# imaranresearch/LAMMPS-SPHERHARM

Measured on AMD Instinct MI355X. Metric: contact_pairs_per_sec, higher is better.
Workload: dtype f64; 1 GPU; BASELINE configs[1]: 100000 particles/GPU, 1 SH shape(s) L_max=6, dense packed bed (jittered HCP, spacing 1.9 mean radii), n_q=16 (Q=512 nodes/pair), pair_coeff kn=1000 exponent=1.25 (overlap volume + force + torque), inputs resident in HBM; particles_per_gpu=100000, lmax=6, nq=16, rule=sharp, backend=none, half_list_pairs_rank0=579574, contact_pairs_rank0=579574, touching_pairs_rank0=502600, contact_pairs_all_ranks=579574

## Files before the change

### lammps-spherharm_amd/csrc/contact_kernel_azimuth.hpp

```cpp
#pragma once
#include "contact_plan.hpp"
#include "jpoly.hpp"
#include "pair_params.hpp"
#include "pair_rotate.hpp"
#include "ring_tables.hpp"
#include "wave_ops.hpp"

namespace shp {


template <int L, bool NEEDV, int WPP = 1, bool SPEC = false>
__global__ void __launch_bounds__(64 * kMaxWavesPerBlock, SHP_JMIN_WAVES(L, NEEDV, WPP)) pair_contact_azimuth_kernel(const PairParams P)
{
  static_assert(L >= 0, "per-azimuth kernels: compiled orders only");
  constexpr int LJ = L;
  static_assert(!SPEC || (PairSpec<LJ>::nq > 0 && PairSpec<LJ>::wpp == WPP),
                "specialised instances: the orders PairSpec names");
  static_assert(WPP == 1 || WPP == 2, "one or two waves per pair");
  extern __shared__ __attribute__((aligned(16))) unsigned char smem_raw[];
  int lane = threadIdx.x & 63;
  const int wib = __builtin_amdgcn_readfirstlane((int)(threadIdx.x >> 6));
  const int w = P.slot0 + ((WPP == 2) ? (int)blockIdx.x : __builtin_amdgcn_readfirstlane((int)(blockIdx.x * P.waves_per_block)) + wib);
  const int half = (WPP == 2) ? wib : 0;
  const int tid = lane + 64 * half;
  constexpr int NT = 64 * WPP;
  if (w >= P.npairs) return;
  const int LL = L;
  typedef PairSpec<L> Spec;
  const int nq = SPEC ? Spec::nq : P.nq;
  const int P_ring_rows = SPEC ? Spec::rr : P.ring_rows;
  const int P_qcap = SPEC ? Spec::qc : P.qcap;
  constexpr bool CARRY = SHP_CARRY_NODE(L, WPP);
  WaveLdsLayout W = (WPP == 2) ? pair_lds_layout2(LL, P_ring_rows, nq, P_qcap)
                               : wave_lds_layout(LL, P_ring_rows, false, nq, P_qcap);
  if constexpr (WPP == 2) {
    W.qri += half * W.qstride;
    W.qrj += half * W.qstride;
    W.qp += half * W.qstride;
    W.park += half * W.qstride;
  }
  typedef __attribute__((address_space(3))) unsigned char lds_byte_t;
  const unsigned wave_off = (WPP == 2) ? 0u : (unsigned)(wib * P.wave_lds_bytes);
  const unsigned wave_abs = __builtin_amdgcn_readfirstlane((unsigned)(size_t)(lds_byte_t*)smem_raw + wave_off);
#define WAVE_LDS() ((double*)(lds_byte_t*)(size_t)launder_s32(wave_abs))
  double* lw = WAVE_LDS();

  __builtin_amdgcn_s_setprio(3);
  const int* rid = P.rec_i + 4 * (size_t)w;
  constexpr int NSL = ((L + 1) * (L + 1) + NT - 1) / NT;
  double vi[NSL], vj[NSL];
  JPolyPre<LJ> pre;
  const double recv = P.rec[(size_t)kRecStride * w + (lane < kRecUsed ? lane : 0)];
  {
    constexpr int ns = (L + 1) * (L + 1);
#pragma unroll
    for (int t = 0; t < NSL; ++t) {
      const int e = tid + NT * t;
      const int ec = e < ns ? e : 0;
      if constexpr (rot_tiled(L)) {
        const int l = (int)__builtin_amdgcn_sqrtf((float)ec + 0.5f);
        const double* tile = P.rot + (size_t)((2 * w) >> 6) * rot_tile_doubles(L);
        const unsigned at = 64u * (unsigned)(l * l) + (unsigned)((2 * w) & 63) * (unsigned)(2 * l + 1) + (unsigned)(ec - l * l);
        vi[t] = tile[at];
        vj[t] = tile[at + (unsigned)(2 * l + 1)];
      } else {
        const size_t at = (size_t)(2 * w) * rot_row_doubles(L) + ec;
        vi[t] = P.rot[at];
        vj[t] = P.rot[at + rot_row_doubles(L)];
      }
    }
    pre.fetch(P, lane, nq);
  }
  double glt_first = 0.0, glw_first = 0.0;
  glw_first = P.glw[tid < nq ? tid : 0];
  if constexpr (L <= 8 && WPP == 1) {
    const int nr0 = P_ring_rows < nq ? P_ring_rows : nq;
    const int lg0 = ring_poly_map(nr0, L + 1, 64);
    const int kr = lg0 >= 1 ? (lane >> lg0) : lane / (L + 1);
    glt_first = P.glt[kr < nr0 ? kr : nr0 - 1];
  }
  const int status = rid[0];
  if (status == 0) return;
  double s_rho = 0.0, s_rj = 0.0, s_rj2 = 0.0, s_rho2 = 0.0, s_pj = 0.0, s_tol1 = 0.0, s_tol3 = 0.0, s_tiny = 0.0;
  {
    const cdptr rs = launder_uniform(P.rec + (size_t)kRecStride * w);
    s_rho = rs[FR_RHO];
    s_rj = rs[FR_RJ];
    s_rj2 = rs[FR_RJ2];
    s_rho2 = rs[FR_RHO2];
    s_pj = rs[FR_JPJ];
    s_tol1 = rs[FR_JTOL1];
    s_tol3 = rs[FR_JTOL3];
    s_tiny = rs[FR_JTINY];
  }
  const bool centre_in_bj = rid[3] != 0;
  if ((tid >= 12 && tid < 30) || (tid >= 36 && tid < kRecUsed)) lw[frj(tid)] = recv;
  if constexpr (L <= 8 && WPP == 1) lw[W.stash + lane] = glt_first;
#pragma unroll
  for (int t = 0; t < NSL; ++t)
    if (tid + NT * t < (LJ + 1) * (LJ + 1)) {
      lw[W.v0 + tid + NT * t] = vj[t];
      lw[W.v0i + tid + NT * t] = vi[t];
    }
  pair_sync<WPP>();
#if defined(SHP_ABL) && SHP_ABL == 1
  asm volatile("" ::"v"(lw[lane & 31]));
  return;
#endif
  jpoly_build<LJ, WPP>(P, lw, W, lane, nq, pre, glw_first, half);
#if defined(SHP_ABL) && SHP_ABL == 4
  asm volatile("" ::"v"(lw[W.pi + lane]));
  return;
#endif

  const double* fr = WAVE_LDS();

  bool centre_inside = false;
  if (NEEDV && centre_in_bj) {
    const double rho = fr[frj(FR_RHO)];
    const double rj = jpoly_eval<LJ>(fr + W.gh, -1.0, 0.0);
    centre_inside = (rho - rj <= 0.0);
  }

  const int npsi = 2 * nq;
  const unsigned magic = ((1u << 24) + (unsigned)npsi - 1u) / (unsigned)npsi;
  const int per_ring = nq / WPP;
  const unsigned magicr = ((1u << 24) + (unsigned)per_ring - 1u) / (unsigned)per_ring;
  const int nslabs = (nq * per_ring + 63) >> 6;
  const int rowlen = 4 * (LL + 1);

  {
    const int kend0 = (P_ring_rows < nq) ? P_ring_rows : nq;
    cap_frame_rings_poly<LJ, WPP>(P, WAVE_LDS(), W, lane, tid, 0, kend0, fr[frj(FR_HW)], fr[frj(FR_HM)], L <= 8 && WPP == 1);
  }
  bool first_group = true;
  double aV = 0.0, aS0 = 0.0, aS1 = 0.0, aS2 = 0.0, aT0 = 0.0, aT1 = 0.0, aT2 = 0.0;
#if defined(SHP_ABL) && SHP_ABL == 3
  int qhead = 0;
#endif
  int qcount = 0, slab = 0;

  while (slab < nslabs) {
  const int sfirst = slab;
  const int k0 = (int)(((unsigned)(sfirst << 6) * magicr) >> 24);
  const int kend = (k0 + P_ring_rows < nq) ? k0 + P_ring_rows : nq;
  const int slab_end = (kend == nq) ? nslabs : ((kend * per_ring) >> 6);
  if (slab_end <= slab) return;
  __builtin_amdgcn_s_setprio(3);
  {
    double* lr = WAVE_LDS();
    if (!first_group) {
      double* park = lr + W.park + lane;
      park[0] = aT2; park[64] = NEEDV ? aV : aS0;
      if constexpr (WPP == 2) __syncthreads();
      cap_frame_rings_poly<LJ, WPP>(P, lr, W, lane, tid, k0, kend - k0, lr[frj(FR_HW)], lr[frj(FR_HM)], false);
      park = WAVE_LDS() + W.park + lane;
      aT2 = park[0];
      if (NEEDV) aV = park[64]; else aS0 = park[64];
      wave_lds_sync();
    }
    first_group = false;
#if defined(SHP_ABL) && SHP_ABL == 2
    asm volatile("" ::"v"(lr[W.ring + lane]));
    return;
#endif
  }

  auto phase2 = [&](auto dir_c, const int dp, const double dri, const double drj, const unsigned long long mdir)
                    __attribute__((always_inline)) {
    constexpr bool DIR = decltype(dir_c)::value;
    (void)dp; (void)dri; (void)drj; (void)mdir;
    wave_lds_sync();
    fr = WAVE_LDS();
    const int cnt = DIR ? 64 : (qcount < 64 ? qcount : 64);
    const bool active = DIR ? lane_of(mdir) : lane < cnt;
    if constexpr (!DIR) qcount -= cnt;
    const int e = DIR ? 0 : qcount + min(lane, cnt - 1);
#ifdef SHP_STATS
    if (lane == 0) atomicAdd(&P.dbg[4], 1ULL);
    if (active) atomicAdd(&P.dbg[7], 1ULL);
#endif
    int p;
    double ri;
    if constexpr (DIR) {
      p = dp;
      ri = dri;
    } else {
      p = ((const unsigned short*)(fr + W.qp))[e];
      ri = fr[W.qri + e];
    }
    int k = (int)(umul_sel<true>((unsigned)p, magic) >> 24);
    int l = p - mul_sel<true>(k, npsi);
    double omi = active ? fr[frj(FR_WSC)] * fr[W.glw + mul_sel<true>(k, jpoly_row(LJ))] : 0.0;
    double c1 = P.cpsi[l], s1 = P.spsi[l];
    double mu, sig;
    {
      const double* row = fr + W.ring + (k - k0) * rowlen;
      mu = row[1];
      sig = row[3];
    }

    double rin = 0.0;
    if (NEEDV) {
      const double rj0 = DIR ? drj : fr[W.qrj + e];
      double uj0, uj1;
      const int ghrow_ = W.gh + mul_sel<true>(l >= nq ? l - nq : l, jpoly_row(LJ));
      uj0 = mu;
      uj1 = (l >= nq) ? -sig : sig;
      double lo = 0.0, hi = ri, lam, xa = ri, ga, xb = ri, gb;
      {
        double bp, s2i;
        {
          const double rho = s_rho;
          bp = mu * rho;
          const double q0 = fma(ri, uj0, -rho), q1 = ri * uj1;
          s2i = fma(q0, q0, q1 * q1);
        }
        const double rho2l = s_rho2;
        if (!centre_in_bj) lo = bp - sqrt_nr1<true>(fma(bp, bp, -s_pj));
        lam = bp - sqrt_nr1<true>(fma(bp, bp, -(rho2l - rj0 * rj0)));
        if (!(lam > lo && lam < hi)) lam = 0.5 * (lo + hi);
        ga = gb = sqrt_nr1<true>(s2i) - rj0;
      }
      unsigned jrow_addr = wave_abs + 8u * (unsigned)ghrow_;
      unsigned long long mact;
      mact = centre_inside ? 0ULL : (DIR ? mdir : (cnt >= 64 ? ~0ULL : ((1ULL << cnt) - 1ULL)));
      auto iterate = [&](double& xa, double& ga, const double xb, const double gb, const double lam, double& gc,
                         const bool have3) __attribute__((always_inline)) {
#ifdef SHP_STATS
        if (lane == 0) atomicAdd(&P.dbg[5], 1ULL);
        if (lane_of(mact)) atomicAdd(&P.dbg[6], 1ULL);
#endif
        double y0, y1, ss2;
        y0 = fma(lam, uj0, -s_rho);
        y1 = lam * uj1;
        ss2 = fma(y0, y0, y1 * y1);
        const bool z0 = !(ss2 > 0.0);
        const double iv = rsqrt_nr1(ss2);
        double rj;
        jrow_addr = launder_u32(jrow_addr);
        rj = jpoly_eval<LJ>((const double*)(lds_byte_t*)(size_t)jrow_addr, y0 * iv, y1 * iv);
        const double Rjl = s_rj;
        double gl = ss2 * iv - rj;
        if (wave_any(z0)) {
          asm volatile("; rare: a point on x_j");
          gl = z0 ? -Rjl : gl;
        }
        {
          const bool pos = gl >= 0.0;
          lo = pos ? lam : lo;
          hi = pos ? hi : lam;
          const double dbl = gb - gl;
          double ext;
          if (!have3) {
            ext = fma(gl * (lam - xb), rcp_nr1(dbl), lam);
          } else {
            const double dab = ga - gb, dal = ga - gl;
            const double num = fma(xa * gb, gl * dbl, fma(lam * ga, gb * dab, -(xb * ga) * (gl * dal)));
            ext = num * rcp_nr1(dab * dal * dbl);
          }
          const bool inb = ext > lo && ext < hi;
          const bool accept = fabs(gl) <= (have3 ? s_tol3 : s_tol1);
          const bool tiny = hi - lo <= s_tiny;
          double res = ext, nxt = ext;
          unsigned long long mstop = wave_ballot(accept);
          if (mask_any(mact & (wave_ballot(tiny) | ~(wave_ballot(ext > lo) & wave_ballot(ext < hi))))) {
#ifdef SHP_STATS
            if (lane == 0) atomicAdd(&P.dbg[8], 1ULL);
#endif
            double sec = ext, e2 = ext;
            if (have3) {
              const double s2 = fma(gl * (lam - xb), rcp_nr1(dbl), lam);
              const bool fin0 = fabs(ext) <= 1e300;
              sec = (!fin0 || !inb) ? s2 : ext;
              e2 = fin0 ? ext : s2;
            }
            const double mid = 0.5 * (lo + hi);
            double n2 = (e2 > lo && e2 < hi) ? e2 : sec;
            n2 = (n2 > lo && n2 < hi) ? n2 : mid;
            const double accv = (fabs(e2) <= 1e300) ? fmin(fmax(e2, lo), hi) : lam;
            res = accept ? accv : (tiny ? mid : n2);
            nxt = n2;
            mstop |= wave_ballot(tiny);
          }
          rin = lane_of(mact) ? res : rin;
          mact &= ~mstop;
          gc = gl;
          xa = nxt;
        }
      };
      double gl0 = 0.0;
      if constexpr (SHP_PEEL(L)) {
      do {
        if (!mask_any(mact)) break;
        iterate(xa, ga, xb, gb, lam, gl0, false);
        if (!mask_any(mact)) break;
        iterate(xb, gb, lam, gl0, xa, ga, true);
        if (!mask_any(mact)) break;
        iterate(lam, gl0, xa, ga, xb, gb, true);
        for (int it = 3; it < 60; it = __builtin_amdgcn_readfirstlane(it + 3)) {
          if (!mask_any(mact)) break;
          iterate(xa, ga, xb, gb, lam, gl0, true);
          if (!mask_any(mact)) break;
          iterate(xb, gb, lam, gl0, xa, ga, true);
          if (!mask_any(mact)) break;
          iterate(lam, gl0, xa, ga, xb, gb, true);
        }
      } while (false);
      } else {
      for (int it = 0; it < 60; it = __builtin_amdgcn_readfirstlane(it + 3)) {
        if (!mask_any(mact)) break;
        iterate(xa, ga, xb, gb, lam, gl0, it >= 1);
        if (!mask_any(mact)) break;
        iterate(xb, gb, lam, gl0, xa, ga, true);
        if (!mask_any(mact)) break;
        iterate(lam, gl0, xa, ga, xb, gb, true);
      }
      }
      auto ri_again = [&]() __attribute__((always_inline)) {
        const int lrow = l >= nq ? l - nq : l;
        const double* tgd = jpoly_trig_sep(LJ) ? fr + W.tr + 2 * lrow : fr + W.gh + mul_sel<true>(lrow, jpoly_row(LJ)) + jpoly_trig(LJ);
        double cd = 1.0, sd = 0.0;
        if constexpr (LJ >= 1) {
          const v2d csd = lds2(tgd);
          const double sgd = (l >= nq) ? -1.0 : 1.0;
          cd = sgd * csd[0];
          sd = sgd * csd[1];
        }
        return ring_value<LJ>(fr + W.ring + (k - k0) * rowlen, cd, sd);
      };
      if constexpr (!CARRY) {
        if constexpr (!DIR) {
          const int e2 = (int)launder_u32((unsigned)e);
          ri = fr[W.qri + e2];
          p = ((const unsigned short*)(fr + W.qp))[e2];
        }
        p = (int)launder_u32((unsigned)p);
        k = (int)(umul_sel<true>((unsigned)p, magic) >> 24);
        l = p - mul_sel<true>(k, npsi);
        omi = active ? fr[frj(FR_WSC)] * fr[W.glw + mul_sel<true>(k, jpoly_row(LJ))] : 0.0;
        const double* row = fr + W.ring + (k - k0) * rowlen;
        mu = row[1];
        sig = row[3];
        if constexpr (DIR) ri = ri_again();
      } else {
        if constexpr (DIR) {
          ri = ri_again();
        } else {
          const int e2 = (int)launder_u32((unsigned)e);
          ri = fr[W.qri + e2];
        }
      }
      const double dv3 = ri * ri * ri - rin * rin * rin;
      aV = fma(omi * (1.0 / 3.0), dv3, aV);
    }

    fr = WAVE_LDS();
    double rmu, rpsi;
    {
      const double sg = (l >= nq) ? -1.0 : 1.0;
      const int lrow = l >= nq ? l - nq : l;
      const double* tg = jpoly_trig_sep(LJ) ? fr + W.tr + 2 * lrow : fr + W.gh + mul_sel<true>(lrow, jpoly_row(LJ)) + jpoly_trig(LJ);
      if constexpr (LJ >= 1) {
        const v2d cs1 = lds2(tg);
        c1 = sg * cs1[0];
        s1 = sg * cs1[1];
      }
      ring_grad_rec<LJ>(fr + W.ring + (k - k0) * rowlen, c1, s1, rmu, rpsi);
    }
    const double rad = ri * fma(ri, sig, rmu * sig * mu);
    const double tan_ = ri * rpsi * rcp_nr1(sig);
    const double A0 = fma(rad, c1, tan_ * s1);
    const double A1 = fma(rad, s1, -tan_ * c1);
    const double A2 = ri * fma(ri, mu, -(sig * sig) * rmu);
    aS0 = fma(omi, A0, aS0);
    aS1 = fma(omi, A1, aS1);
    aS2 = fma(omi, A2, aS2);
    const double wr = omi * ri;
    const double u0 = sig * c1, u1 = sig * s1;
    aT0 = fma(wr, u1 * A2 - mu * A1, aT0);
    aT1 = fma(wr, mu * A0 - u0 * A2, aT1);
    aT2 = fma(wr, u0 * A1 - u1 * A0, aT2);
    wave_lds_sync();
  };
  __builtin_amdgcn_s_setprio(0);
  for (;;) {
#define SHP_PUSH(m_, pn, rin_, rjn_)                                                                                  \
    {                                                                                                                  \
      if (m_ != 0ULL) {                                                                                                \
        if (lane_of(m_)) {                                                                                             \
          const int pos_ = qcount + (int)__builtin_amdgcn_mbcnt_hi((unsigned)(m_ >> 32),                               \
                                                    __builtin_amdgcn_mbcnt_lo((unsigned)m_, 0u));                      \
          double* lq_ = WAVE_LDS();                                                                                     \
          ((unsigned short*)(lq_ + W.qp))[pos_] = (unsigned short)(pn);                                                \
          lq_[W.qri + pos_] = (rin_);                                                                                  \
          lq_[W.qrj + pos_] = (rjn_);                                                                                  \
        }                                                                                                              \
        qcount += __builtin_popcountll(m_);                                                                            \
      }                                                                                                                \
    }
    while (qcount < 64 && slab < slab_end) {
      fr = WAVE_LDS();
      const int pp = (slab << 6) + lane;
      const int ppc = min(pp, nq * per_ring - 1);
      const int k = (int)(umul_sel<true>((unsigned)ppc, magicr) >> 24);
      const int l = ppc - mul_sel<true>(k, per_ring) + half * per_ring;
      const double* row = fr + W.ring + (k - k0) * rowlen;
      const v2d r01 = lds2(row);
      const double mu = r01[1], sig = row[3];
      const double* gr = fr + W.gh + mul_sel<true>(l, jpoly_row(LJ));
      double re = r01[0], ro = 0.0;
      if constexpr (LJ >= 1) {
        const v2d cs1 = lds2(jpoly_trig_sep(LJ) ? fr + W.tr + 2 * l : gr + jpoly_trig(LJ));
        const double c1 = cs1[0], s1 = cs1[1];
        double cm = c1, sm = s1, cp = 1.0, sp = 0.0;
        const double tc = c1 + c1;
#pragma unroll
        for (int m = 1; m <= LJ; ++m) {
          const v2d ab = lds2(row + 4 * m);
          const double A = ab[0], B = ab[1];
          if (m & 1) ro = fma(A, cm, fma(B, sm, ro));
          else re = fma(A, cm, fma(B, sm, re));
          if (m < LJ) {
            const double c = fma(tc, cm, -cp), s = fma(tc, sm, -sp);
            cp = cm;
            sp = sm;
            cm = c;
            sm = s;
          }
        }
      }
      const double ria = re + ro, rib = re - ro;
      const double rho = s_rho, rj2 = s_rj2;
      const double qa0 = fma(ria, mu, -rho), qa1 = ria * sig;
      const double qb0 = fma(rib, mu, -rho), qb1 = -rib * sig;
      const double sa2 = fma(qa0, qa0, qa1 * qa1), sb2 = fma(qb0, qb0, qb1 * qb1);
      const int nvalid = nq * per_ring - (slab << 6);
      const unsigned long long mvalid = nvalid >= 64 ? ~0ULL : ((1ULL << nvalid) - 1ULL);
      const unsigned long long mca = wave_ballot(sa2 < rj2) & mvalid, mcb = wave_ballot(sb2 < rj2) & mvalid;
      if ((mca | mcb) == 0ULL) {
#ifdef SHP_STATS
        if (lane == 0) atomicAdd(&P.dbg[0], 2ULL);
#endif
        ++slab;
        continue;
      }
      const bool za = !(sa2 > 0.0), zb = !(sb2 > 0.0);
      const unsigned long long mza = wave_ballot(za), mzb = wave_ballot(zb);
      const double inva = rsqrt_nr1(sa2), invb = rsqrt_nr1(sb2);
      double rjae, rjbe;
      jpoly_eval2<LJ>(fr + W.gh + mul_sel<true>(l, jpoly_row(LJ)), qa0 * inva, qa1 * inva, qb0 * invb, qb1 * invb, rjae, rjbe);
      const double Rjl = s_rj;
      double rja = rjae, rjb = rjbe;
      if (mask_any(mza | mzb)) {
        asm volatile("; rare: a node on x_j");
        rja = za ? Rjl : rjae;
        rjb = zb ? Rjl : rjbe;
      }
      const unsigned long long ma = mca & (mza | wave_ballot(sa2 * inva < rja));
      const unsigned long long mb = mcb & (mzb | wave_ballot(sb2 * invb < rjb));
      const int pa = mul_sel<true>(k, npsi) + l;
#ifdef SHP_STATS
      if (qcount + __builtin_popcountll(ma) + __builtin_popcountll(mb) > W.qcap) {
        if (lane == 0) atomicAdd(&P.dbg[9], 1ULL);
      }
#endif
      if (qcount + __builtin_popcountll(ma) + __builtin_popcountll(mb) > W.qcap) {
        const unsigned long long mboth = ma & mb;
        SHP_PUSH(mboth, pa, ria, rja);
        const bool second = lane_of(mb);
        ++slab;
#ifdef SHP_STATS
        if (lane == 0) atomicAdd(&P.dbg[0], 2ULL);
        if (lane_of(mca)) atomicAdd(&P.dbg[1], 1ULL);
        if (lane_of(mcb)) atomicAdd(&P.dbg[1], 1ULL);
        if (lane == 0) atomicAdd(&P.dbg[2], 2ULL);
        if (lane_of(ma)) atomicAdd(&P.dbg[3], 1ULL);
        if (lane_of(mb)) atomicAdd(&P.dbg[3], 1ULL);
        if (lane == 0) atomicAdd(&P.dbg[10], 1ULL);
        if (lane == 0 && P.dbg[15]) atomicAdd(&P.dbg[64 + w], (unsigned long long)(__builtin_popcountll(ma) + __builtin_popcountll(mb)));
#endif
        phase2(BoolC<true>{}, second ? pa + nq : pa, second ? rib : ria, second ? rjb : rja, ma | mb);
        continue;
      }
#ifdef SHP_STATS
      if (lane == 0) atomicAdd(&P.dbg[0], 2ULL);
      if (lane_of(mca)) atomicAdd(&P.dbg[1], 1ULL);
      if (lane_of(mcb)) atomicAdd(&P.dbg[1], 1ULL);
      if (lane == 0) atomicAdd(&P.dbg[2], 2ULL);
      if (lane_of(ma)) atomicAdd(&P.dbg[3], 1ULL);
      if (lane_of(mb)) atomicAdd(&P.dbg[3], 1ULL);
      if (lane == 0 && P.dbg[15]) atomicAdd(&P.dbg[64 + w], (unsigned long long)(__builtin_popcountll(ma) + __builtin_popcountll(mb)));
#endif
      ++slab;
      SHP_PUSH(ma, pa, ria, rja);
      SHP_PUSH(mb, pa + nq, rib, rjb);
    }
#undef SHP_PUSH
    if (qcount == 0) break;
#if defined(SHP_ABL) && SHP_ABL == 3
    qhead = (qhead + qcount) & (kQueue - 1);
    qcount = 0;
    continue;
#endif

    phase2(BoolC<false>{}, 0, 0.0, 0.0, 0ULL);
  }
  }

  __builtin_amdgcn_s_setprio(3);
  lane = fresh_lane();
  if constexpr (WPP == 2) __syncthreads();
  {
    double* red = WAVE_LDS() + ((WPP == 2 && half) ? (int)(P.wave_lds_bytes >> 3) - kRedPerWave : kFrameJ);
    red[0 * kRedStride + lane] = aS0; red[1 * kRedStride + lane] = aS1; red[2 * kRedStride + lane] = aS2;
    red[3 * kRedStride + lane] = aT0; red[4 * kRedStride + lane] = aT1; red[5 * kRedStride + lane] = aT2;
    red[6 * kRedStride + lane] = NEEDV ? aV : 0.0;
    wave_lds_sync();
    double* part = red + 7 * kRedStride;
    if (lane < 56) {
      const double* src = red + (lane >> 3) * kRedStride + (lane & 7);
      part[lane] = ((src[0] + src[8]) + (src[16] + src[24])) + ((src[32] + src[40]) + (src[48] + src[56]));
    }
    wave_lds_sync();
    double* tot = part + 56;
    if (lane < 7) {
      const double* src = part + 8 * lane;
      tot[lane] = ((src[0] + src[1]) + (src[2] + src[3])) + ((src[4] + src[5]) + (src[6] + src[7]));
    }
    wave_lds_sync();
    if constexpr (WPP == 2) {
      __syncthreads();
      if (half != 0) return;
      if (lane < 7) tot[lane] += WAVE_LDS()[(int)(P.wave_lds_bytes >> 3) - kRedPerWave + 7 * kRedStride + 56 + lane];
      wave_lds_sync();
    }
  }
  if (lane >= 6) return;
  fr = WAVE_LDS();
  const double* tot = fr + kFrameJ + 7 * kRedStride + 56;
  double* fcomp = (double*)tot + 7;
  const int comp = (lane >= 3) ? lane - 3 : lane;
  const bool is_t = lane >= 3;
  const double a0 = tot[is_t ? 3 : 0], a1 = tot[is_t ? 4 : 1], a2 = tot[is_t ? 5 : 2];
  const double val = fr[frj(FR_E1) + comp] * a0 + fr[frj(FR_E2) + comp] * a1 + fr[frj(FR_C) + comp] * a2;
  const double aVt = tot[6];

  LateParams& E = *late_params();
  if (E.pair_out) {
    double* o = E.pair_out + 7 * (size_t)w;
    o[1 + lane] = val;
    if (lane == 0) o[0] = aVt;
  }
  const bool touched = NEEDV ? (aVt > 0.0) : (wave_ballot(!is_t && val != 0.0) != 0ULL);
  if (E.flags && lane == 0) E.flags[w] = touched ? 2 : 1;
  if (!touched) return;

  const int* ij = (const int*)(fr + frj(FR_IJ));
  const int i = ij[0], j = ij[1];
  const double knij = fr[frj(FR_KN)], mij = fr[frj(FR_EXPO)];
  const double vm1 = (mij == 1.0) ? 1.0 : pow_quarter(aVt, mij - 1.0);
  const double pn = knij * mij * vm1;
  const double Fm = -pn * val;
  fcomp[lane] = Fm;
  wave_lds_sync();
  double* const det = E.pair_ft;
  if (det) det[12 * (size_t)w + lane] = Fm;
  else atomicAdd((is_t ? E.torque : E.f) + 3 * (size_t)i + comp, Fm);
  const bool applyj = E.newton_pair || j < E.nlocal;
  if (applyj) {
    const int c1 = (comp == 2) ? 0 : comp + 1, c2 = (comp == 0) ? 2 : comp - 1;
    double vj = -Fm;
    if (is_t) vj -= fr[frj(FR_D) + c1] * (-fcomp[c2]) - fr[frj(FR_D) + c2] * (-fcomp[c1]);
    if (det) det[12 * (size_t)w + 6 + lane] = vj;
    else atomicAdd((is_t ? E.torque : E.f) + 3 * (size_t)j + comp, vj);
  }
  if ((E.eflag || E.vflag) && E.pair_ev) {
    const double share = E.newton_pair ? 1.0 : (0.5 + (j < E.nlocal ? 0.5 : 0.0));
    double* row = E.pair_ev + 8 * (size_t)w;
    if (E.vflag) {
      const int a = (lane < 3) ? lane : ((lane == 5) ? 1 : 0);
      const int b = (lane < 3) ? lane : ((lane == 3) ? 1 : 2);
      row[1 + lane] = share * (-fr[frj(FR_D) + a]) * fcomp[b];
    }
    if (E.eflag && lane == 0) row[0] = share * knij * (vm1 * aVt);
  }
  if (lane != 0) return;
  if (E.eatom || E.vatom) {
    const double F0 = fcomp[0], F1 = fcomp[1], F2 = fcomp[2];
    const double d0 = fr[frj(FR_D)], d1 = fr[frj(FR_D) + 1], d2 = fr[frj(FR_D) + 2];
    const bool owni = E.newton_pair || i < E.nlocal;
    if (E.eatom) {
      const double eh = 0.5 * knij * (vm1 * aVt);
      if (owni) atomicAdd(&E.eatom[i], eh);
      if (applyj) atomicAdd(&E.eatom[j], eh);
    }
    if (E.vatom) {
      const double v[6] = {0.5 * (-d0) * F0, 0.5 * (-d1) * F1, 0.5 * (-d2) * F2,
                           0.5 * (-d0) * F1, 0.5 * (-d0) * F2, 0.5 * (-d1) * F2};
      for (int a = 0; a < 6; ++a) {
        if (owni) atomicAdd(&E.vatom[6 * (size_t)i + a], v[a]);
        if (applyj) atomicAdd(&E.vatom[6 * (size_t)j + a], v[a]);
      }
    }
  }
}
#undef WAVE_LDS

}
```

### lammps-spherharm_amd/csrc/pair_kernel.hpp

```cpp
#pragma once
#include "contact_plan.hpp"
#include "pair_params.hpp"
#include "pair_rotate.hpp"

#ifndef SHP_WMIN_WAVES
#define SHP_WMIN_WAVES(L) (((L) >= 0 && (L) <= 6 && (L) != 3) ? 5 : 4)
#endif
#ifndef SHP_MIN_WAVES
#define SHP_MIN_WAVES(L, NEEDV) \
  ((NEEDV) ? (((L) == 0 || (L) == 1 || (L) == 6) ? 6 : 5) : (((L) >= 0 && (L) <= 6) ? 6 : 5))
#endif
#ifndef SHP_JMIN_WAVES
#define SHP_JMIN_WAVES(L, NEEDV, WPP) (((L) <= 4) ? 6 : (((L) <= 6 || ((L) == 9 && (WPP) == 1 && !(NEEDV))) ? 5 : 4))
#endif

#ifndef SHP_PEEL
#define SHP_PEEL(L) ((L) >= 6)
#endif
#ifndef SHP_CARRY_NODE
#define SHP_CARRY_NODE(L, WPP) ((L) >= 6 && !((L) == 9 && (WPP) == 1))
#endif

namespace shp {
template <bool B>
struct BoolC { static constexpr bool value = B; };
}

#include "contact_kernel_azimuth.hpp"
#include "contact_kernel_body.hpp"

namespace shp {

template <int L, bool AZIMUTH = false, int WPP = 1, bool SPEC = false>
const void* contact_kernel(const bool needv)
{
  if constexpr (AZIMUTH)
    return needv ? (const void*)pair_contact_azimuth_kernel<L, true, WPP, SPEC>
                 : (const void*)pair_contact_azimuth_kernel<L, false, WPP, SPEC>;
  else
    return needv ? (const void*)pair_contact_body_kernel<L, true>
                 : (const void*)pair_contact_body_kernel<L, false>;
}
template <int L>
const void* pair_contact_instance(const ContactPlan& p, const bool needv)
{
  if constexpr (L >= 0) {
    if (p.weighted) return (const void*)pair_contact_body_kernel<L, true, true>;
    if constexpr (PairSpec<L>::nq > 0)
      if (p.spec) return contact_kernel<L, true, PairSpec<L>::wpp, true>(needv);
    if constexpr (split_compiled(L))
      if (p.waves_per_pair == 2) return contact_kernel<L, true, 2>(needv);
    if (p.family == 1) return contact_kernel<L, true>(needv);
  }
  return contact_kernel<L>(needv);
}

template <int L>
void launch_pair_contact(const PairParams& P, const ContactPlan& plan, bool needv, hipStream_t st, hipEvent_t wait_before_contact)
{
  const int nslots = P.npairs - P.slot0;
  if (nslots <= 0) return;
  if constexpr (L >= 0) {
    if (plan.family == 1)
      hipLaunchKernelGGL((pair_rotate_lane_kernel<L>), dim3((2 * (unsigned)nslots + 63) / 64), dim3(64),
                         RotLaneLds<L>::bytes(), st, P, const_cast<double*>(P.rot));
  }
  if (wait_before_contact) (void)hipStreamWaitEvent(st, wait_before_contact, 0);
  const int wpb = plan.waves_per_block;
  const size_t lds = (size_t)wpb * plan.lds_bytes;
  const void* kern = pair_contact_instance<L>(plan, needv);
  if (lds > 65536) (void)hipFuncSetAttribute(kern, hipFuncAttributeMaxDynamicSharedMemorySize, (int)lds);
  void* args[] = {const_cast<PairParams*>(&P)};
  (void)hipLaunchKernel(kern, dim3((nslots + wpb - 1) / wpb), dim3(64 * wpb * plan.waves_per_pair), args, lds, st);
}

}
```

### lammps-spherharm_amd/csrc/ring_tables.hpp

```cpp
#pragma once
#include "contact_plan.hpp"
#include "sh_const.hpp"
#include "wave_ops.hpp"

namespace shp {

template <int L, int WPP, bool DENSE>
__device__ __forceinline__ void ring_lane_map(const int lane, const int nrows, int& krl, int& g, int& G, int& rpc, int& lg)
{
  const int lg1 = (nrows <= 8) ? 3 : (nrows <= 16) ? 2 : (nrows <= 32) ? 1 : 0;
  lg = lg1 + (WPP == 2 ? 1 : 0);
  G = 1 << lg;
  krl = lane >> lg;
  g = lane & (G - 1);
  rpc = (64 * WPP) >> lg;
  if constexpr (DENSE && L >= 1 && WPP == 1) {
    if ((L + 1) * nrows <= 64) {
      G = L + 1;
      krl = lane / (L + 1);
      g = lane - krl * (L + 1);
      rpc = 64 / (L + 1);
      lg = 0;
    }
  }
}

template <int L, bool PRE = false, int WPP = 1, bool DENSE = false>
__device__ __forceinline__ void cap_frame_rings(const PairParams& P, double* __restrict__ lw, const WaveLdsLayout& W,
                                                const int LL, const int lane, const int k0, const int nrows,
                                                const double hw, const double hm, const bool have_first = false)
{
  const double* ch = lw + W.v0;
  double* ring = lw + W.ring;
  int krl, g, G, rpc, lg;
  ring_lane_map<L, WPP, DENSE>(lane, nrows, krl, g, G, rpc, lg);
  for (int kr0 = 0; kr0 < nrows; kr0 += rpc) {
    const int kr = kr0 + krl;
    const bool row_ok = kr < nrows && krl < rpc;
    const double tk = (PRE && have_first && k0 == 0 && kr0 == 0) ? lw[W.stash + lane] : P.glt[k0 + (row_ok ? kr : 0)];
    const double mu = fma(hw, tk, hm);
    const double sig2 = fmax(0.0, fma(-mu, mu, 1.0));
    const double sig = sqrt_nr(sig2);
    double sp = 1.0, sigG = sig;
    for (int t = 0; t < G - 1; ++t) {
      if (t < g) sp *= sig;
    }
    for (int t = 0; t < lg; ++t) sigG *= sigG;
    for (int m0 = 0; m0 <= LL; m0 += G) {
      const int m = m0 + g;
      const bool ok = row_ok && m <= LL;
      const int mc = ok ? m : 0;
      const double* rcm = P.rc + (sh_moff(LL, mc) - mc);
      const double* cp = ch + mc;
      const double* cm = ch - mc;
      const bool modd = (mc & 1) != 0;
      double qe = modd ? 0.0 : 1.0, qo = modd ? 1.0 : 0.0, de = 0.0, dd = 0.0;
      double wa = cp[mc * mc + mc], wb = cm[mc * mc + mc], wad = 0.0, wbd = 0.0;
      constexpr int NPRE = (PRE && L >= 1) ? L : 1;
      double pa[NPRE];
      if constexpr (PRE && L >= 1) {
#pragma unroll
        for (int n = 1; n <= L; ++n) {
          if (n <= m0) continue;
          pa[n - 1] = rcm[n];
        }
#pragma unroll
        for (int n = 1; n <= L; ++n) {
          if (n <= m0) continue;
          asm volatile("" : "+v"(pa[n - 1]));
        }
      }
#pragma unroll
      for (int n = 1; n <= ((L >= 0) ? L : LL); ++n) {
        if (n <= m0) continue;
        if (ok && n > m) {
          const double a = (PRE && L >= 1) ? pa[(PRE && L >= 1) ? n - 1 : 0] : rcm[n];
          const double ca = cp[n * n + n], cbm = cm[n * n + n];
          if (n & 1) {
            dd = fma(a, fma(mu, de, qe), -dd);
            qo = fma(a, mu * qe, -qo);
            wa = fma(ca, qo, wa); wb = fma(cbm, qo, wb); wad = fma(ca, dd, wad); wbd = fma(cbm, dd, wbd);
          } else {
            de = fma(a, fma(mu, dd, qo), -de);
            qe = fma(a, mu * qo, -qe);
            wa = fma(ca, qe, wa); wb = fma(cbm, qe, wb); wad = fma(ca, de, wad); wbd = fma(cbm, de, wbd);
          }
        }
      }
      if (ok) {
        const double f = (m > 0) ? (double)m * mu * rcp_nr(sig2) : 0.0;
        double* o = ring + 4 * (kr * (LL + 1) + m);
        o[0] = sp * wa;
        o[2] = sp * fma(-f, wa, wad);
        if (m == 0) {
          o[1] = mu;
          o[3] = sig;
        } else {
          o[1] = sp * wb;
          o[3] = sp * fma(-f, wb, wbd);
        }
      }
      sp *= sigG;
    }
  }
  pair_sync<WPP>();
}

__host__ __device__ inline int ring_poly_map(const int nrows, const int K, const int NT)
{
  const int nent = nrows * K;
  if (nent <= NT) return -1;
  int lg = 0;
  while ((NT >> (lg + 1)) >= nrows && (1 << lg) < K) ++lg;
  if (lg < 1) return -1;
  const int E = (K + (1 << lg) - 1) >> lg, passes = (nent + NT - 1) / NT;
  return (25 + 44 * E < 69 * passes) ? lg : -1;
}

template <int L, int WPP, class PP = PairParams>
__device__ __forceinline__ void cap_frame_rings_poly(const PP& P, double* __restrict__ lw, const WaveLdsLayout& W,
                                                     const int lane, const int tid, const int k0, const int nrows,
                                                     const double hw, const double hm, const bool have_first)
{
  constexpr int K = L + 1, NT = 64 * WPP;
  const double* pi = lw + W.pi;
  double* ring = lw + W.ring;
  const int nent = nrows * K;
  const int lg = ring_poly_map(nrows, K, NT);
  auto entry = [&](const int m, const int e, const bool store, const double mu, const double sig, const double isig)
                   __attribute__((always_inline)) {
    const double* row = pi + (2 * K) * m;
    v2d c[K];
#pragma unroll
    for (int t = 0; t < K; ++t) c[t] = lds2(row + 2 * t);
#define SHP_EL(j) c[(j) >> 1][(j) & 1]
    double pc = SHP_EL(L), ps = SHP_EL(K + L), dc = 0.0, ds = 0.0;
    if constexpr (L >= 1) {
      dc = pc;
      ds = ps;
      pc = fma(pc, mu, SHP_EL(L - 1));
      ps = fma(ps, mu, SHP_EL(K + L - 1));
#pragma unroll
      for (int q = L - 2; q >= 0; --q) {
        dc = fma(dc, mu, pc);
        ds = fma(ds, mu, ps);
        pc = fma(pc, mu, SHP_EL(q));
        ps = fma(ps, mu, SHP_EL(K + q));
      }
    }
#undef SHP_EL
    const bool odd = (m & 1) != 0;
    const double sm = odd ? sig : 1.0;
    const double tm = odd ? -mu * isig : 0.0;
    const double A = sm * pc, dA = fma(tm, pc, sm * dc);
    double B = sm * ps, dB = fma(tm, ps, sm * ds);
    if (m == 0) {
      B = mu;
      dB = sig;
    }
    if (store) {
      double* o = ring + 4 * e;
      *(v2d*)__builtin_assume_aligned(o, 16) = v2d{A, B};
      *(v2d*)__builtin_assume_aligned(o + 2, 16) = v2d{dA, dB};
    }
  };
  if (lg >= 1) {
    const int G = 1 << lg, kr = tid >> lg, g = tid & (G - 1);
    const int krc = min(kr, nrows - 1);
    const double tk = (have_first && k0 == 0) ? lw[W.stash + lane] : P.glt[k0 + krc];
    const double mu = fma(hw, tk, hm);
    const double sig2 = max_raw(fma(-mu, mu, 1.0), 1e-300);
    const double isig = rsqrt_nr(sig2);
    const double sig = sig2 * isig;
    for (int m0 = 0; m0 < K; m0 += G) {
      const int m = m0 + g;
      entry(min(m, K - 1), krc * K + m, kr < nrows && m < K, mu, sig, isig);
    }
  } else {
    for (int e0 = 0; e0 < nent; e0 += NT) {
      const int e = e0 + tid;
      const int ec = min(e, nent - 1);
      const int kr = (int)((unsigned)ec / (unsigned)K), m = ec - kr * K;
      const double tk = (have_first && k0 == 0 && e0 == 0) ? lw[W.stash + lane] : P.glt[k0 + kr];
      const double mu = fma(hw, tk, hm);
      const double sig2 = max_raw(fma(-mu, mu, 1.0), 1e-300);
      const double isig = rsqrt_nr(sig2);
      const double sig = sig2 * isig;
      entry(m, e, e < nent, mu, sig, isig);
    }
  }
  pair_sync<WPP>();
}

__host__ __device__ constexpr bool trig_lmajor(int L) { return L >= 2 && L <= 6; }

struct QuadLayout {
  int lmax, npsi, nm;
  size_t glt, glw, cpsi, spsi, trig, trigj, size;
  int trig_stride;
  QuadLayout(const int L, const int nq)
      : lmax(L), npsi(2 * nq), nm(L >= 2 ? L - 1 : 0), glt(0), glw(nq), cpsi(2 * (size_t)nq), spsi(4 * (size_t)nq),
        trig(6 * (size_t)nq), trigj(trig + (size_t)nm * 2 * npsi), size(trigj + (size_t)nq * (L + 2) * 2),
        trig_stride(trig_lmajor(L) ? 2 * (L - 1) : 4 * nq)
  {
  }
  size_t trig_at(const int l, const int m) const
  {
    return trig + 2 * (trig_lmajor(lmax) ? ((size_t)l * nm + (m - 2)) : ((size_t)(m - 2) * npsi + l));
  }
  size_t trigj_at(const int l, const int m) const { return trigj + ((size_t)l * (lmax + 2) + m) * 2; }
};

template <int L, bool GRAD>
__device__ __forceinline__ void ring_eval(const double* __restrict__ row, const int LL, const double c1, const double s1,
                                          const double* __restrict__ tr, const int tstride, double& r, double& rmu,
                                          double& rpsi)
{
  r = row[0];
  rmu = GRAD ? row[2] : 0.0;
  rpsi = 0.0;
  double cm = c1, sm = s1;
  const int lim = (L >= 0) ? L : LL;
#pragma unroll
  for (int m = 1; m <= lim; ++m) {
    if (L >= 2 && m >= 2) {
      cm = tr[trig_lmajor(L) ? 2 * (m - 2) : (m - 2) * tstride];
      sm = tr[(trig_lmajor(L) ? 2 * (m - 2) : (m - 2) * tstride) + 1];
    }
    const v2d ab = lds2(row + 4 * m);
    const double A = ab[0], B = ab[1];
    r = fma(A, cm, r);
    r = fma(B, sm, r);
    if (GRAD) {
      const v2d dab = lds2(row + 4 * m + 2);
      rmu = fma(dab[0], cm, rmu);
      rmu = fma(dab[1], sm, rmu);
      const double dm = (double)m;
      rpsi = fma(dm * B, cm, rpsi);
      rpsi = fma(-dm * A, sm, rpsi);
    }
    if (L < 2 && m < lim) {
      const double c = fma(cm, c1, -(sm * s1)), s = fma(cm, s1, sm * c1);
      cm = c;
      sm = s;
    }
  }
}

}
```

Before: 259.8 million contact-pairs/s.

## Fuse surface force/torque accumulation into phase-1 ring scan for high orders

For L>=6 (except L=12 split-wave), the surface integrand for force and torque is computed directly in the phase-1 azimuth scan. It uses a new shared even/odd ring recurrence that gives both psi and psi+pi nodes at once. When the overlap volume is not needed, the queue push and phase-2 pass are skipped entirely. When it is needed, phase 2 only does the volume root-find and no longer recomputes the ring gradient. This removes queue traffic, the ring recomputation and extra LDS syncs, but adds gradient work to every touching node in phase 1 and may raise register pressure.

Measured after the change: 263.5 million contact-pairs/s (median of 6 runs). 1.4% higher.

```diff
diff --git a/lammps-spherharm_amd/csrc/contact_kernel_azimuth.hpp b/lammps-spherharm_amd/csrc/contact_kernel_azimuth.hpp
--- a/lammps-spherharm_amd/csrc/contact_kernel_azimuth.hpp
+++ b/lammps-spherharm_amd/csrc/contact_kernel_azimuth.hpp
@@ -30,7 +30,8 @@
   const int nq = SPEC ? Spec::nq : P.nq;
   const int P_ring_rows = SPEC ? Spec::rr : P.ring_rows;
   const int P_qcap = SPEC ? Spec::qc : P.qcap;
-  constexpr bool CARRY = SHP_CARRY_NODE(L, WPP);
+  constexpr bool P1S = SHP_SURFACE_PHASE1(L, NEEDV, WPP);
+  constexpr bool CARRY = !P1S && SHP_CARRY_NODE(L, WPP);
   WaveLdsLayout W = (WPP == 2) ? pair_lds_layout2(LL, P_ring_rows, nq, P_qcap)
                                : wave_lds_layout(LL, P_ring_rows, false, nq, P_qcap);
   if constexpr (WPP == 2) {
@@ -166,6 +167,22 @@
 #endif
   }
 
+  auto surface = [&](const double ri, const double rmu, const double rpsi, const double c, const double s, const double mu,
+                     const double sig, const double isig, const double omi) __attribute__((always_inline)) {
+    const double rad = ri * fma(ri, sig, rmu * sig * mu);
+    const double tan_ = ri * rpsi * isig;
+    const double A0 = fma(rad, c, tan_ * s);
+    const double A1 = fma(rad, s, -tan_ * c);
+    const double A2 = ri * fma(ri, mu, -(sig * sig) * rmu);
+    aS0 = fma(omi, A0, aS0);
+    aS1 = fma(omi, A1, aS1);
+    aS2 = fma(omi, A2, aS2);
+    const double wr = omi * ri;
+    const double u0 = sig * c, u1 = sig * s;
+    aT0 = fma(wr, u1 * A2 - mu * A1, aT0);
+    aT1 = fma(wr, mu * A0 - u0 * A2, aT1);
+    aT2 = fma(wr, u0 * A1 - u1 * A0, aT2);
+  };
   auto phase2 = [&](auto dir_c, const int dp, const double dri, const double drj, const unsigned long long mdir)
                     __attribute__((always_inline)) {
     constexpr bool DIR = decltype(dir_c)::value;
@@ -192,7 +209,12 @@
     int k = (int)(umul_sel<true>((unsigned)p, magic) >> 24);
     int l = p - mul_sel<true>(k, npsi);
     double omi = active ? fr[frj(FR_WSC)] * fr[W.glw + mul_sel<true>(k, jpoly_row(LJ))] : 0.0;
-    double c1 = P.cpsi[l], s1 = P.spsi[l];
+    const double omi3 = omi * (1.0 / 3.0);
+    double c1 = 0.0, s1 = 0.0;
+    if constexpr (!P1S) {
+      c1 = P.cpsi[l];
+      s1 = P.spsi[l];
+    }
     double mu, sig;
     {
       const double* row = fr + W.ring + (k - k0) * rowlen;
@@ -317,47 +339,54 @@
         iterate(lam, gl0, xa, ga, xb, gb, true);
       }
       }
-      auto ri_again = [&]() __attribute__((always_inline)) {
-        const int lrow = l >= nq ? l - nq : l;
-        const double* tgd = jpoly_trig_sep(LJ) ? fr + W.tr + 2 * lrow : fr + W.gh + mul_sel<true>(lrow, jpoly_row(LJ)) + jpoly_trig(LJ);
-        double cd = 1.0, sd = 0.0;
-        if constexpr (LJ >= 1) {
-          const v2d csd = lds2(tgd);
-          const double sgd = (l >= nq) ? -1.0 : 1.0;
-          cd = sgd * csd[0];
-          sd = sgd * csd[1];
+      if constexpr (P1S) {
+        if constexpr (!DIR) ri = fr[W.qri + (int)launder_u32((unsigned)e)];
+        const double dv3 = ri * ri * ri - rin * rin * rin;
+        aV = fma(omi3, dv3, aV);
+      } else {
+        auto ri_again = [&]() __attribute__((always_inline)) {
+          const int lrow = l >= nq ? l - nq : l;
+          const double* tgd = jpoly_trig_sep(LJ) ? fr + W.tr + 2 * lrow : fr + W.gh + mul_sel<true>(lrow, jpoly_row(LJ)) + jpoly_trig(LJ);
+          double cd = 1.0, sd = 0.0;
+          if constexpr (LJ >= 1) {
+            const v2d csd = lds2(tgd);
+            const double sgd = (l >= nq) ? -1.0 : 1.0;
+            cd = sgd * csd[0];
+            sd = sgd * csd[1];
+          }
+          return ring_value<LJ>(fr + W.ring + (k - k0) * rowlen, cd, sd);
+        };
+        if constexpr (!CARRY) {
+          if constexpr (!DIR) {
+            const int e2 = (int)launder_u32((unsigned)e);
+            ri = fr[W.qri + e2];
+            p = ((const unsigned short*)(fr + W.qp))[e2];
+          }
+          p = (int)launder_u32((unsigned)p);
+          k = (int)(umul_sel<true>((unsigned)p, magic) >> 24);
+          l = p - mul_sel<true>(k, npsi);
+          omi = active ? fr[frj(FR_WSC)] * fr[W.glw + mul_sel<true>(k, jpoly_row(LJ))] : 0.0;
+          const double* row = fr + W.ring + (k - k0) * rowlen;
+          mu = row[1];
+          sig = row[3];
+          if constexpr (DIR) ri = ri_again();
+        } else {
+          if constexpr (DIR) {
+            ri = ri_again();
+          } else {
+            const int e2 = (int)launder_u32((unsigned)e);
+            ri = fr[W.qri + e2];
+          }
         }
-        return ring_value<LJ>(fr + W.ring + (k - k0) * rowlen, cd, sd);
-      };
-      if constexpr (!CARRY) {
-        if constexpr (!DIR) {
-          const int e2 = (int)launder_u32((unsigned)e);
-          ri = fr[W.qri + e2];
-          p = ((const unsigned short*)(fr + W.qp))[e2];
-        }
-        p = (int)launder_u32((unsigned)p);
-        k = (int)(umul_sel<true>((unsigned)p, magic) >> 24);
-        l = p - mul_sel<true>(k, npsi);
-        omi = active ? fr[frj(FR_WSC)] * fr[W.glw + mul_sel<true>(k, jpoly_row(LJ))] : 0.0;
-        const double* row = fr + W.ring + (k - k0) * rowlen;
-        mu = row[1];
-        sig = row[3];
-        if constexpr (DIR) ri = ri_again();
-      } else {
-        if constexpr (DIR) {
-          ri = ri_again();
-        } else {
-          const int e2 = (int)launder_u32((unsigned)e);
-          ri = fr[W.qri + e2];
-        }
-      }
-      const double dv3 = ri * ri * ri - rin * rin * rin;
-      aV = fma(omi * (1.0 / 3.0), dv3, aV);
-    }
-
-    fr = WAVE_LDS();
-    double rmu, rpsi;
-    {
+        const double dv3 = ri * ri * ri - rin * rin * rin;
+        aV = fma(omi * (1.0 / 3.0), dv3, aV);
+      }
+    }
+
+#if !(defined(SHP_ABL) && SHP_ABL == 6)
+    if constexpr (!P1S) {
+      fr = WAVE_LDS();
+      double rmu, rpsi;
       const double sg = (l >= nq) ? -1.0 : 1.0;
       const int lrow = l >= nq ? l - nq : l;
       const double* tg = jpoly_trig_sep(LJ) ? fr + W.tr + 2 * lrow : fr + W.gh + mul_sel<true>(lrow, jpoly_row(LJ)) + jpoly_trig(LJ);
@@ -367,20 +396,9 @@
         s1 = sg * cs1[1];
       }
       ring_grad_rec<LJ>(fr + W.ring + (k - k0) * rowlen, c1, s1, rmu, rpsi);
-    }
-    const double rad = ri * fma(ri, sig, rmu * sig * mu);
-    const double tan_ = ri * rpsi * rcp_nr1(sig);
-    const double A0 = fma(rad, c1, tan_ * s1);
-    const double A1 = fma(rad, s1, -tan_ * c1);
-    const double A2 = ri * fma(ri, mu, -(sig * sig) * rmu);
-    aS0 = fma(omi, A0, aS0);
-    aS1 = fma(omi, A1, aS1);
-    aS2 = fma(omi, A2, aS2);
-    const double wr = omi * ri;
-    const double u0 = sig * c1, u1 = sig * s1;
-    aT0 = fma(wr, u1 * A2 - mu * A1, aT0);
-    aT1 = fma(wr, mu * A0 - u0 * A2, aT1);
-    aT2 = fma(wr, u0 * A1 - u1 * A0, aT2);
+      surface(ri, rmu, rpsi, c1, s1, mu, sig, rcp_nr1(sig), omi);
+    }
+#endif
     wave_lds_sync();
   };
   __builtin_amdgcn_s_setprio(0);
@@ -409,28 +427,16 @@
       const v2d r01 = lds2(row);
       const double mu = r01[1], sig = row[3];
       const double* gr = fr + W.gh + mul_sel<true>(l, jpoly_row(LJ));
-      double re = r01[0], ro = 0.0;
-      if constexpr (LJ >= 1) {
-        const v2d cs1 = lds2(jpoly_trig_sep(LJ) ? fr + W.tr + 2 * l : gr + jpoly_trig(LJ));
-        const double c1 = cs1[0], s1 = cs1[1];
-        double cm = c1, sm = s1, cp = 1.0, sp = 0.0;
-        const double tc = c1 + c1;
-#pragma unroll
-        for (int m = 1; m <= LJ; ++m) {
-          const v2d ab = lds2(row + 4 * m);
-          const double A = ab[0], B = ab[1];
-          if (m & 1) ro = fma(A, cm, fma(B, sm, ro));
-          else re = fma(A, cm, fma(B, sm, re));
-          if (m < LJ) {
-            const double c = fma(tc, cm, -cp), s = fma(tc, sm, -sp);
-            cp = cm;
-            sp = sm;
-            cm = c;
-            sm = s;
-          }
+      double ria, rib;
+      {
+        double c1 = 1.0, s1 = 0.0, unused0, unused1;
+        if constexpr (LJ >= 1) {
+          const v2d cs1 = lds2(jpoly_trig_sep(LJ) ? fr + W.tr + 2 * l : gr + jpoly_trig(LJ));
+          c1 = cs1[0];
+          s1 = cs1[1];
         }
-      }
-      const double ria = re + ro, rib = re - ro;
+        ring_pair_rec<LJ, false>(row, r01[0], c1, s1, ria, rib, unused0, unused1);
+      }
       const double rho = s_rho, rj2 = s_rj2;
       const double qa0 = fma(ria, mu, -rho), qa1 = ria * sig;
       const double qb0 = fma(rib, mu, -rho), qb1 = -rib * sig;
@@ -459,6 +465,35 @@
       }
       const unsigned long long ma = mca & (mza | wave_ballot(sa2 * inva < rja));
       const unsigned long long mb = mcb & (mzb | wave_ballot(sb2 * invb < rjb));
+#if !(defined(SHP_ABL) && SHP_ABL == 6)
+      if (P1S && (ma | mb) != 0ULL) {
+        static_assert(!P1S || LJ >= 1, "the trig of the first order comes from particle j's table");
+        const double* fg = WAVE_LDS();
+        const double* rowg = fg + W.ring + (k - k0) * rowlen;
+        const v2d cs1 = lds2(jpoly_trig_sep(LJ) ? fg + W.tr + 2 * l : fg + W.gh + mul_sel<true>(l, jpoly_row(LJ)) + jpoly_trig(LJ));
+        const double c1 = cs1[0], s1 = cs1[1];
+        const v2d g23 = lds2(rowg + 2);
+        const double mug = rowg[1], sigg = g23[1];
+        double rmua, rmub, rpsia, rpsib;
+        ring_pair_rec<LJ, true, SHP_GRAD_CHUNK(L)>(rowg, g23[0], c1, s1, rmua, rmub, rpsia, rpsib);
+        const double om = fg[frj(FR_WSC)] * fg[W.glw + mul_sel<true>(k, jpoly_row(LJ))];
+        const double isig = rcp_nr1(sigg);
+        surface(ria, rmua, rpsia, c1, s1, mug, sigg, isig, lane_of(ma) ? om : 0.0);
+        surface(rib, rmub, rpsib, -c1, -s1, mug, sigg, isig, lane_of(mb) ? om : 0.0);
+      }
+#endif
+      if constexpr (P1S && !NEEDV) {
+#ifdef SHP_STATS
+        if (lane == 0) atomicAdd(&P.dbg[0], 2ULL);
+        if (lane_of(mca)) atomicAdd(&P.dbg[1], 1ULL);
+        if (lane_of(mcb)) atomicAdd(&P.dbg[1], 1ULL);
+        if (lane == 0) atomicAdd(&P.dbg[2], 2ULL);
+        if (lane_of(ma)) atomicAdd(&P.dbg[3], 1ULL);
+        if (lane_of(mb)) atomicAdd(&P.dbg[3], 1ULL);
+#endif
+        ++slab;
+        continue;
+      }
       const int pa = mul_sel<true>(k, npsi) + l;
 #ifdef SHP_STATS
       if (qcount + __builtin_popcountll(ma) + __builtin_popcountll(mb) > W.qcap) {
@@ -497,7 +532,7 @@
       SHP_PUSH(mb, pa + nq, rib, rjb);
     }
 #undef SHP_PUSH
-    if (qcount == 0) break;
+    if ((P1S && !NEEDV) || qcount == 0) break;
 #if defined(SHP_ABL) && SHP_ABL == 3
     qhead = (qhead + qcount) & (kQueue - 1);
     qcount = 0;
diff --git a/lammps-spherharm_amd/csrc/pair_kernel.hpp b/lammps-spherharm_amd/csrc/pair_kernel.hpp
--- a/lammps-spherharm_amd/csrc/pair_kernel.hpp
+++ b/lammps-spherharm_amd/csrc/pair_kernel.hpp
@@ -19,6 +19,12 @@
 #endif
 #ifndef SHP_CARRY_NODE
 #define SHP_CARRY_NODE(L, WPP) ((L) >= 6 && !((L) == 9 && (WPP) == 1))
+#endif
+#ifndef SHP_SURFACE_PHASE1
+#define SHP_SURFACE_PHASE1(L, NEEDV, WPP) ((L) >= 6 && !((L) == 12 && (WPP) == 2))
+#endif
+#ifndef SHP_GRAD_CHUNK
+#define SHP_GRAD_CHUNK(L) ((L) >= 7 ? 1 : 0)
 #endif
 
 namespace shp {
diff --git a/lammps-spherharm_amd/csrc/ring_tables.hpp b/lammps-spherharm_amd/csrc/ring_tables.hpp
--- a/lammps-spherharm_amd/csrc/ring_tables.hpp
+++ b/lammps-spherharm_amd/csrc/ring_tables.hpp
@@ -247,4 +247,53 @@
   }
 }
 
-}
+template <int L, bool GRAD, int CHUNK = 0>
+__device__ __forceinline__ void ring_pair_rec(const double* __restrict__ row0, const double a0, const double c1, const double s1,
+                                              double& va, double& vb, double& wa, double& wb)
+{
+  double ve = a0, vo = 0.0, we = 0.0, wo = 0.0;
+  const double* row = row0;
+  if constexpr (L >= 1) {
+    double cm = c1, sm = s1, cp = 1.0, sp = 0.0;
+    const double tc = c1 + c1;
+#pragma unroll
+    for (int m = 1; m <= L; ++m) {
+      const v2d ab = lds2(row + 4 * m);
+      const double A = ab[0], B = ab[1];
+      if constexpr (!GRAD) {
+        if (m & 1) vo = fma(A, cm, fma(B, sm, vo));
+        else ve = fma(A, cm, fma(B, sm, ve));
+      } else {
+        const v2d dab = lds2(row + 4 * m + 2);
+        const double t = fma(B, cm, -(A * sm)), dm = (double)m;
+        if (m & 1) {
+          vo = fma(dab[0], cm, fma(dab[1], sm, vo));
+          wo = (m == 1) ? t : fma(dm, t, wo);
+        } else {
+          ve = fma(dab[0], cm, fma(dab[1], sm, ve));
+          we = (m == 2) ? dm * t : fma(dm, t, we);
+        }
+      }
+      if (m < L) {
+        const double c = fma(tc, cm, -cp), s = fma(tc, sm, -sp);
+        cp = cm;
+        sp = sm;
+        cm = c;
+        sm = s;
+        if constexpr (GRAD && CHUNK > 0) {
+          if (m % CHUNK == 0) {
+            unsigned ra_ = (unsigned)(size_t)(const __attribute__((address_space(3))) double*)row;
+            asm volatile("" : "+v"(ra_), "+v"(ve), "+v"(vo), "+v"(cm), "+v"(sm));
+            row = (const double*)(const __attribute__((address_space(3))) double*)(size_t)ra_;
+          }
+        }
+      }
+    }
+  }
+  va = ve + vo;
+  vb = ve - vo;
+  wa = we + wo;
+  wb = we - wo;
+}
+
+}
```
